# ShangHua-Gao/SOD100K

Measured on NVIDIA H100. Metric: images/sec CSNet fwd 224x224, higher is better.
Workload: dtype fp16

## Files before the change

### sod100k_b200/csrc/il_stream.cuh

```cuda
#pragma once
#include <cuda.h>

#include "il_block.cuh"

namespace csnet {

constexpr int kIlsMaxThreads = 768;
constexpr int kIlsMaxC = 64;
constexpr int kIlsHiStages = 2, kIlsLoStages = 3;

struct IlsArgs {
  void* yh;
  void* yl;
  const uint32_t* wh;
  const uint32_t* wl;
  DwParams dw1h, dw1l, dw2h, dw2l;
  float bias_h[kIlsMaxC], sm1_h[kIlsMaxC], bias_l[kIlsMaxC], sm1_l[kIlsMaxC];
  int32_t N, H, W;
  int32_t Chi, Cli, Cho, Clo;
  int32_t K8, K16, NH, NL;
  int32_t SH, SL, ST;
  int32_t GH, GL;
  int32_t ns, gsn, hl;
  int32_t GR, GLR;
  int32_t Ci, BW;
  int32_t off_xlo;
  int32_t cpi, total_chunks;
  int32_t dw_warps;
  int32_t hi_stage_bytes, lo_stage_bytes;
  int32_t off_xl, off_xh, off_t1l, off_wbh, off_wbl, off_bar, off_zero, off_epi, smem_bytes;
};

__device__ __forceinline__ void tma_load_5d(uint32_t dst, const CUtensorMap* tm, uint32_t bar, int c0, int c1, int c2, int c3, int c4) {
  asm volatile("cp.async.bulk.tensor.5d.shared::cluster.global.mbarrier::complete_tx::bytes [%0], [%1, {%3, %4, %5, %6, %7}], [%2];\n"
               ::"r"(dst), "l"(tm), "r"(bar), "r"(c0), "r"(c1), "r"(c2), "r"(c3), "r"(c4) : "memory");
}
__device__ __forceinline__ void tma_load_4d_a(uint32_t dst, const CUtensorMap* tm, uint32_t bar, int c0, int c1, int c2, int c3) {
  asm volatile("cp.async.bulk.tensor.4d.shared::cluster.global.mbarrier::complete_tx::bytes [%0], [%1, {%3, %4, %5, %6}], [%2];\n"
               ::"r"(dst), "l"(tm), "r"(bar), "r"(c0), "r"(c1), "r"(c2), "r"(c3) : "memory");
}
__device__ __forceinline__ void mbar_expect_tx_a(uint32_t bar, uint32_t bytes) {
  asm volatile("mbarrier.arrive.expect_tx.shared::cta.b64 _, [%0], %1;\n" ::"r"(bar), "r"(bytes) : "memory");
}
__device__ __forceinline__ void mbar_wait_a(uint32_t bar, uint32_t parity) {
  uint32_t ok = 0;
  const long long t0 = clock64();
  while (true) {
    asm volatile("{\n.reg .pred p;\nmbarrier.try_wait.parity.shared::cta.b64 p, [%1], %2;\nselp.u32 %0, 1, 0, p;\n}\n"
                 : "=r"(ok) : "r"(bar), "r"(parity) : "memory");
    if (ok) break;
    if (clock64() - t0 > 4000000000LL) __trap();
  }
}
__device__ __forceinline__ uint64_t gmma_desc(uint32_t saddr, uint32_t lbo_bytes, uint32_t sbo_bytes) {
  return (uint64_t)((saddr & 0x3FFFF) >> 4) | ((uint64_t)((lbo_bytes >> 4) & 0x3FFF) << 16) |
         ((uint64_t)((sbo_bytes >> 4) & 0x3FFF) << 32);
}
template <int N> struct Wgmma;
template <> struct Wgmma<16> {
  static __device__ __forceinline__ void mma(float (&d)[8], uint64_t da, uint64_t db, uint32_t acc) {
    asm volatile("{\n.reg .pred p;\nsetp.ne.b32 p, %10, 0;\n"
                 "wgmma.mma_async.sync.aligned.m64n16k16.f32.f16.f16 {%0, %1, %2, %3, %4, %5, %6, %7}, %8, %9, p, 1, 1, 1, 0;\n}\n"
                 : "+f"(d[0]), "+f"(d[1]), "+f"(d[2]), "+f"(d[3]), "+f"(d[4]), "+f"(d[5]), "+f"(d[6]), "+f"(d[7])
                 : "l"(da), "l"(db), "r"(acc));
  }
};
template <> struct Wgmma<32> {
  static __device__ __forceinline__ void mma(float (&d)[16], uint64_t da, uint64_t db, uint32_t acc) {
    asm volatile("{\n.reg .pred p;\nsetp.ne.b32 p, %18, 0;\n"
                 "wgmma.mma_async.sync.aligned.m64n32k16.f32.f16.f16 {%0, %1, %2, %3, %4, %5, %6, %7, %8, %9, %10, %11, %12, %13, %14, %15}, %16, %17, p, 1, 1, 1, 0;\n}\n"
                 : "+f"(d[0]), "+f"(d[1]), "+f"(d[2]), "+f"(d[3]), "+f"(d[4]), "+f"(d[5]), "+f"(d[6]), "+f"(d[7]), "+f"(d[8]), "+f"(d[9]), "+f"(d[10]), "+f"(d[11]), "+f"(d[12]), "+f"(d[13]), "+f"(d[14]), "+f"(d[15])
                 : "l"(da), "l"(db), "r"(acc));
  }
};
template <> struct Wgmma<48> {
  static __device__ __forceinline__ void mma(float (&d)[24], uint64_t da, uint64_t db, uint32_t acc) {
    asm volatile("{\n.reg .pred p;\nsetp.ne.b32 p, %26, 0;\n"
                 "wgmma.mma_async.sync.aligned.m64n48k16.f32.f16.f16 {%0, %1, %2, %3, %4, %5, %6, %7, %8, %9, %10, %11, %12, %13, %14, %15, %16, %17, %18, %19, %20, %21, %22, %23}, %24, %25, p, 1, 1, 1, 0;\n}\n"
                 : "+f"(d[0]), "+f"(d[1]), "+f"(d[2]), "+f"(d[3]), "+f"(d[4]), "+f"(d[5]), "+f"(d[6]), "+f"(d[7]), "+f"(d[8]), "+f"(d[9]), "+f"(d[10]), "+f"(d[11]), "+f"(d[12]), "+f"(d[13]), "+f"(d[14]), "+f"(d[15]), "+f"(d[16]), "+f"(d[17]), "+f"(d[18]), "+f"(d[19]), "+f"(d[20]), "+f"(d[21]), "+f"(d[22]), "+f"(d[23])
                 : "l"(da), "l"(db), "r"(acc));
  }
};
template <> struct Wgmma<64> {
  static __device__ __forceinline__ void mma(float (&d)[32], uint64_t da, uint64_t db, uint32_t acc) {
    asm volatile("{\n.reg .pred p;\nsetp.ne.b32 p, %34, 0;\n"
                 "wgmma.mma_async.sync.aligned.m64n64k16.f32.f16.f16 {%0, %1, %2, %3, %4, %5, %6, %7, %8, %9, %10, %11, %12, %13, %14, %15, %16, %17, %18, %19, %20, %21, %22, %23, %24, %25, %26, %27, %28, %29, %30, %31}, %32, %33, p, 1, 1, 1, 0;\n}\n"
                 : "+f"(d[0]), "+f"(d[1]), "+f"(d[2]), "+f"(d[3]), "+f"(d[4]), "+f"(d[5]), "+f"(d[6]), "+f"(d[7]), "+f"(d[8]), "+f"(d[9]), "+f"(d[10]), "+f"(d[11]), "+f"(d[12]), "+f"(d[13]), "+f"(d[14]), "+f"(d[15]), "+f"(d[16]), "+f"(d[17]), "+f"(d[18]), "+f"(d[19]), "+f"(d[20]), "+f"(d[21]), "+f"(d[22]), "+f"(d[23]), "+f"(d[24]), "+f"(d[25]), "+f"(d[26]), "+f"(d[27]), "+f"(d[28]), "+f"(d[29]), "+f"(d[30]), "+f"(d[31])
                 : "l"(da), "l"(db), "r"(acc));
  }
};
template <> struct Wgmma<80> {
  static __device__ __forceinline__ void mma(float (&d)[40], uint64_t da, uint64_t db, uint32_t acc) {
    asm volatile("{\n.reg .pred p;\nsetp.ne.b32 p, %42, 0;\n"
                 "wgmma.mma_async.sync.aligned.m64n80k16.f32.f16.f16 {%0, %1, %2, %3, %4, %5, %6, %7, %8, %9, %10, %11, %12, %13, %14, %15, %16, %17, %18, %19, %20, %21, %22, %23, %24, %25, %26, %27, %28, %29, %30, %31, %32, %33, %34, %35, %36, %37, %38, %39}, %40, %41, p, 1, 1, 1, 0;\n}\n"
                 : "+f"(d[0]), "+f"(d[1]), "+f"(d[2]), "+f"(d[3]), "+f"(d[4]), "+f"(d[5]), "+f"(d[6]), "+f"(d[7]), "+f"(d[8]), "+f"(d[9]), "+f"(d[10]), "+f"(d[11]), "+f"(d[12]), "+f"(d[13]), "+f"(d[14]), "+f"(d[15]), "+f"(d[16]), "+f"(d[17]), "+f"(d[18]), "+f"(d[19]), "+f"(d[20]), "+f"(d[21]), "+f"(d[22]), "+f"(d[23]), "+f"(d[24]), "+f"(d[25]), "+f"(d[26]), "+f"(d[27]), "+f"(d[28]), "+f"(d[29]), "+f"(d[30]), "+f"(d[31]), "+f"(d[32]), "+f"(d[33]), "+f"(d[34]), "+f"(d[35]), "+f"(d[36]), "+f"(d[37]), "+f"(d[38]), "+f"(d[39])
                 : "l"(da), "l"(db), "r"(acc));
  }
};
__device__ __forceinline__ void wgmma_fence() { asm volatile("wgmma.fence.sync.aligned;\n" ::: "memory"); }
__device__ __forceinline__ void wgmma_commit_wait() {
  asm volatile("wgmma.commit_group.sync.aligned;\n" ::: "memory");
  asm volatile("wgmma.wait_group.sync.aligned 0;\n" ::: "memory");
}
__device__ __forceinline__ void warpgroup_bar(int wg) { asm volatile("bar.sync %0, 128;\n" ::"r"(1 + wg) : "memory"); }
template <int N>
__device__ __forceinline__ void wgmma_block(float (&d)[N / 2], uint64_t da, uint64_t db, int K16) {
#pragma unroll
  for (int i = 0; i < N / 2; ++i) d[i] = 0.f;
  wgmma_fence();
  for (int ks = 0; ks < (K16 >> 4); ++ks) Wgmma<N>::mma(d, da + (uint64_t)(16 * ks), db + (uint64_t)(16 * ks), ks > 0);
  wgmma_commit_wait();
}
__device__ __forceinline__ uint32_t lds32(uint32_t a) { uint32_t v; asm volatile("ld.shared.b32 %0, [%1];\n" : "=r"(v) : "r"(a)); return v; }
__device__ __forceinline__ uint2 lds64(uint32_t a) { uint2 v; asm volatile("ld.shared.v2.b32 {%0, %1}, [%2];\n" : "=r"(v.x), "=r"(v.y) : "r"(a)); return v; }
__device__ __forceinline__ uint4 lds128(uint32_t a) {
  uint4 v;
  asm volatile("ld.shared.v4.b32 {%0, %1, %2, %3}, [%4];\n" : "=r"(v.x), "=r"(v.y), "=r"(v.z), "=r"(v.w) : "r"(a));
  return v;
}
__device__ __forceinline__ uint16_t lds16(uint32_t a) { uint16_t v; asm volatile("ld.shared.u16 %0, [%1];\n" : "=h"(v) : "r"(a)); return v; }
__device__ __forceinline__ void sts128(uint32_t a, uint4 v) {
  asm volatile("st.shared.v4.b32 [%0], {%1, %2, %3, %4};\n" ::"r"(a), "r"(v.x), "r"(v.y), "r"(v.z), "r"(v.w) : "memory");
}
__device__ __forceinline__ void sts16(uint32_t a, uint16_t v) { asm volatile("st.shared.u16 [%0], %1;\n" ::"r"(a), "h"(v) : "memory"); }

__device__ __forceinline__ uint16_t h16(const uint32_t* row, int j) { return (j & 1) ? (uint16_t)(row[j >> 1] >> 16) : (uint16_t)row[j >> 1]; }

template <typename T>
__device__ __forceinline__ void ils_dw_push(uint32_t (&t1)[2][6], uint32_t (&t2)[2][5], const uint32_t (&n1)[6],
                                            const uint32_t (&w1)[5], float b1, float s1, const uint32_t (&w2)[5], float b2, float s2,
                                            bool make_t2, float mL, float mR, bool make_out, uint16_t* out) {
  uint32_t q[5];
  if (make_t2) {
#pragma unroll
    for (int i = 0; i < 10; i += 2) {
      float v0 = b1, v1 = b1;
#pragma unroll
      for (int dy = 0; dy < 3; ++dy) {
        const uint32_t* row = dy == 0 ? t1[0] : (dy == 1 ? t1[1] : n1);
#pragma unroll
        for (int dx = 0; dx < 3; ++dx) {
          const uint16_t w = h16(w1, dy * 3 + dx);
          v0 = Pack<T>::fma16(h16(row, i + dx), w, v0);
          v1 = Pack<T>::fma16(h16(row, i + 1 + dx), w, v1);
        }
      }
      v0 = prelu_m1(v0, s1);
      v1 = prelu_m1(v1, s1);
      if (i == 0) v0 *= mL;
      if (i == 8) v1 *= mR;
      q[i >> 1] = Pack<T>::from_f2(v0, v1);
    }
  } else {
#pragma unroll
    for (int i = 0; i < 5; ++i) q[i] = 0u;
  }
  if (make_out) {
    uint32_t o[4];
#pragma unroll
    for (int k = 0; k < 8; k += 2) {
      float v0 = b2, v1 = b2;
#pragma unroll
      for (int dy = 0; dy < 3; ++dy) {
        const uint32_t* row = dy == 0 ? t2[0] : (dy == 1 ? t2[1] : q);
#pragma unroll
        for (int dx = 0; dx < 3; ++dx) {
          const uint16_t w = h16(w2, dy * 3 + dx);
          v0 = Pack<T>::fma16(h16(row, k + dx), w, v0);
          v1 = Pack<T>::fma16(h16(row, k + 1 + dx), w, v1);
        }
      }
      o[k >> 1] = Pack<T>::from_f2(prelu_m1(v0, s2), prelu_m1(v1, s2));
    }
    *reinterpret_cast<uint4*>(out) = make_uint4(o[0], o[1], o[2], o[3]);
  }
#pragma unroll
  for (int i = 0; i < 6; ++i) { t1[0][i] = t1[1][i]; t1[1][i] = n1[i]; }
#pragma unroll
  for (int i = 0; i < 5; ++i) { t2[0][i] = t2[1][i]; t2[1][i] = q[i]; }
}

__device__ __forceinline__ void stsm_x4_trans(uint32_t addr, uint32_t a, uint32_t b, uint32_t c, uint32_t d) {
  asm volatile("stmatrix.sync.aligned.m8n8.x4.trans.shared.b16 [%0], {%1, %2, %3, %4};\n" ::"r"(addr), "r"(a), "r"(b), "r"(c), "r"(d) : "memory");
}

template <typename T, int N>
__device__ __forceinline__ void ils_block(uint64_t da, uint64_t db, int K16, int wg, uint32_t tile, uint32_t gstride, int g0, int ngroups,
                                          uint32_t eb, uint32_t es, uint32_t dummy, int lane) {
  float d[N / 2];
  wgmma_block<N>(d, da, db, K16);
  warpgroup_bar(wg);
  const int q = lane & 3, mrow = lane & 7, mat = lane >> 3;
#pragma unroll
  for (int cc = 0; cc < N / 16; ++cc) {
    const uint32_t co = (uint32_t)(cc * 16 + 2 * q) * 4u;
    const uint2 bA = lds64(eb + co), bB = lds64(eb + co + 32u), sA = lds64(es + co), sB = lds64(es + co + 32u);
    const float b0 = __uint_as_float(bA.x), b1 = __uint_as_float(bA.y), b2 = __uint_as_float(bB.x), b3 = __uint_as_float(bB.y);
    const float s0 = __uint_as_float(sA.x), s1 = __uint_as_float(sA.y), s2 = __uint_as_float(sB.x), s3 = __uint_as_float(sB.y);
    const float* r = d + 8 * cc;
    const uint32_t m0 = Pack<T>::from_f2(prelu_m1(r[0] + b0, s0), prelu_m1(r[1] + b1, s1));
    const uint32_t m1 = Pack<T>::from_f2(prelu_m1(r[2] + b0, s0), prelu_m1(r[3] + b1, s1));
    const uint32_t m2 = Pack<T>::from_f2(prelu_m1(r[4] + b2, s2), prelu_m1(r[5] + b3, s3));
    const uint32_t m3 = Pack<T>::from_f2(prelu_m1(r[6] + b2, s2), prelu_m1(r[7] + b3, s3));
    const int pg = g0 + (mat & 1);
    const uint32_t addr = pg < ngroups ? tile + (uint32_t)pg * gstride + (uint32_t)(cc * 16 + 8 * (mat >> 1) + mrow) * 16u
                                       : dummy + (uint32_t)(mat * 8 + mrow) * 16u;
    stsm_x4_trans(addr, m0, m1, m2, m3);
  }
}
template <typename T>
__device__ __forceinline__ void ils_block_n(int N, uint64_t da, uint64_t db, int K16, int wg, uint32_t tile, uint32_t gstride, int g0,
                                            int ngroups, uint32_t eb, uint32_t es, uint32_t dummy, int lane) {
// ... 26 lines not shown
  if (tid == 0) {
    for (int i = 0; i < 6; ++i) asm volatile("mbarrier.init.shared::cta.b64 [%0], 1;\n" ::"r"(BAR + 8 * i) : "memory");
    asm volatile("fence.mbarrier_init.release.cluster;\n" ::: "memory");
  }
  {
    uint16_t* wb = reinterpret_cast<uint16_t*>(gbase + A.off_wbh);
    const uint16_t* src = reinterpret_cast<const uint16_t*>(A.wh);
    for (int i = tid; i < NH * K16; i += nthreads) {
      const int n = i / K16, k = i - n * K16;
      wb[(((n >> 3) * (K16 >> 3) + (k >> 3)) * 8 + (n & 7)) * 8 + (k & 7)] = k < A.K8 ? src[n * A.K8 + k] : (uint16_t)0;
    }
    if (NL > 0) {
      wb = reinterpret_cast<uint16_t*>(gbase + A.off_wbl);
      src = reinterpret_cast<const uint16_t*>(A.wl);
      for (int i = tid; i < NL * K16; i += nthreads) {
        const int n = i / K16, k = i - n * K16;
        wb[(((n >> 3) * (K16 >> 3) + (k >> 3)) * 8 + (n & 7)) * 8 + (k & 7)] = k < A.K8 ? src[n * A.K8 + k] : (uint16_t)0;
      }
    }
    if (tid < 16) reinterpret_cast<uint32_t*>(gbase + A.off_zero)[tid] = 0u;
    if (kStem) {
      const int per = K16 - Chi, padh = per * 4 * GR, padl = per * 2 * GLR;
      for (int i = tid; i < 2 * padh + padl; i += nthreads) {
        const bool hb = i < 2 * padh;
        const int st = hb ? i / padh : 0, j = hb ? i - st * padh : i - 2 * padh, g_ = j / per, k_ = Chi + (j - g_ * per);
        sts128((hb ? XH + (uint32_t)st * (uint32_t)A.hi_stage_bytes + (uint32_t)(g_ * SH + k_) * 16u
                   : sbase + A.off_xlo + (uint32_t)(g_ * SL + k_) * 16u), make_uint4(0u, 0u, 0u, 0u));
      }
    }
    if (tid < kIlsMaxC) {
      float* ep = reinterpret_cast<float*>(gbase + A.off_epi);
      ep[tid] = A.bias_h[tid]; ep[kIlsMaxC + tid] = A.sm1_h[tid]; ep[2 * kIlsMaxC + tid] = A.bias_l[tid]; ep[3 * kIlsMaxC + tid] = A.sm1_l[tid];
    }
  }
  asm volatile("fence.proxy.async.shared::cta;\n" ::: "memory");
  __syncthreads();

  const int n_hi_tasks = Cho * gsn;
  const bool dw_hi = tid < n_hi_tasks;
  const int dwt = dw_hi ? tid : tid - n_hi_tasks;
  const int Gd = dw_hi ? gsn : gsn >> 1, Cd = dw_hi ? Cho : Clo, Sd = dw_hi ? SH : ST;
  const bool dw_live = dwt < Cd * Gd;
  const int dc = dw_live ? dwt / Gd : 0, dg = dw_live ? dwt - dc * Gd : 0;
  uint32_t w1[5], w2[5];
  float b1, s1, b2, s2;
  {
    const DwParams& P1 = dw_hi ? A.dw1h : A.dw1l;
    const DwParams& P2 = dw_hi ? A.dw2h : A.dw2l;
    float f1[10], f2[10];
#pragma unroll
    for (int i = 0; i < 9; ++i) {
      f1[i] = dw_live ? __ldg(P1.w + dc * 9 + i) : 0.f;
      f2[i] = dw_live ? __ldg(P2.w + dc * 9 + i) : 0.f;
    }
    f1[9] = f2[9] = 0.f;
#pragma unroll
    for (int i = 0; i < 5; ++i) { w1[i] = Pack<T>::from_f2(f1[2 * i], f1[2 * i + 1]); w2[i] = Pack<T>::from_f2(f2[2 * i], f2[2 * i + 1]); }
    b1 = dw_live ? __ldg(P1.b + dc) : 0.f; s1 = dw_live ? __ldg(P1.s + dc) - 1.f : 0.f;
    b2 = dw_live ? __ldg(P2.b + dc) : 0.f; s2 = dw_live ? __ldg(P2.s + dc) - 1.f : 0.f;
  }
  const int dw_rows = dw_hi ? 4 : 2;
  const int dHd = dw_hi ? H : Hl, dWd = dw_hi ? W : Wl;
  const uint32_t dw_off = (uint32_t)((dg + hl) * Sd + dc) * 16u, dw_rowstep = (uint32_t)((dw_hi ? GR : GLR) * Sd) * 16u;
  const int Gimg = dw_hi ? GH : GL;

  const int nbh = (4 * GR + 7) >> 3, nbl = NL > 0 ? (2 * GLR + 7) >> 3 : 0;
  const uint64_t db_h = gmma_desc(WBH, 128u, (uint32_t)(K16 >> 3) * 128u), db_l = gmma_desc(WBL, 128u, (uint32_t)(K16 >> 3) * 128u);
  const uint32_t hi_tx = (uint32_t)(64 * SH * GR), lo_tx = kStem ? (uint32_t)(A.BW * 4 * A.Ci * 4) : (uint32_t)(32 * SL * GLR);
  const uint32_t XLO = sbase + A.off_xlo;

  int ra = (int)((long long)blockIdx.x * A.total_chunks / gridDim.x);
  const int rb = (int)((long long)(blockIdx.x + 1) * A.total_chunks / gridDim.x);
  uint32_t hq = 0, lq = 0;

  while (ra < rb) {
    const int item = ra / cpi, ca = ra - item * cpi;
    const int n = item / A.ns, gs0 = (item - n * A.ns) * gsn;
    const int cb = (ca + (rb - ra)) < cpi ? (ca + (rb - ra)) : cpi;
    ra += cb - ca;
    const int c0 = ca > 0 ? ca - 1 : 0, c1 = cb < cpi ? cb : cpi - 1;
    const int cl0 = c0 > 0 ? c0 - 1 : 0, cl1 = c1 + 1 < cpi ? c1 + 1 : cpi - 1;
    const int out_lo = dw_hi ? 4 * ca : 2 * ca, out_hi = dw_hi ? 4 * cb : 2 * cb;
    const uint32_t hq0 = hq, lq0 = lq;
    hq += (uint32_t)(c1 - c0 + 1);
    lq += (uint32_t)(cl1 - cl0 + 1);
    auto hi_stage = [&](int c) { return XH + ((hq0 + (uint32_t)(c - c0)) & 1u) * (uint32_t)A.hi_stage_bytes; };
    auto lo_stage = [&](int cl) { return XL + ((lq0 + (uint32_t)(cl - cl0)) % 3u) * (uint32_t)A.lo_stage_bytes; };
    auto issue_hi = [&](int c) {
      const uint32_t q = hq0 + (uint32_t)(c - c0), bar = bar_h + 8 * (q & 1u);
      mbar_expect_tx_a(bar, hi_tx);
      tma_load_5d(hi_stage(c), &tmH, bar, 0, 0, gs0 - hl, 4 * c, n);
    };
    auto issue_lo = [&](int cl) {
      const uint32_t q = lq0 + (uint32_t)(cl - cl0), bar = bar_l + 8 * (q % 3u);
      mbar_expect_tx_a(bar, lo_tx);
      if (kStem) tma_load_4d_a(lo_stage(cl), &tmL, bar, 8 * (gs0 - hl) - 4, 4 * cl, 0, n);
      else tma_load_5d(lo_stage(cl), &tmL, bar, 0, 0, (gs0 >> 1) - hl, 2 * cl, n);
    };
    if (tid == 0) {
      asm volatile("fence.proxy.async.shared::cta;\n" ::: "memory");
      if (!kStem) {
        issue_hi(c0);
        if (c0 + 1 <= c1) issue_hi(c0 + 1);
      }
      for (int cl = cl0; cl <= cl1 && cl <= c0 + 1; ++cl) issue_lo(cl);
    }
    int lo_waited = 0;
    uint32_t t1w[2][6], t2w[2][5];
#pragma unroll
    for (int i = 0; i < 6; ++i) t1w[0][i] = t1w[1][i] = 0u;
#pragma unroll
    for (int i = 0; i < 5; ++i) t2w[0][i] = t2w[1][i] = 0u;
    const int gimg = (dw_hi ? gs0 : gs0 >> 1) + dg;
    const bool edgeL = gimg == 0, edgeR = gimg == Gimg - 1;
    const float mL = edgeL ? 0.f : 1.f, mR = edgeR ? 0.f : 1.f;
    uint16_t* ybase = reinterpret_cast<uint16_t*>(dw_hi ? A.yh : A.yl) + ((size_t)n * Cd + dc) * dHd * dWd + 8 * gimg;

    for (int c = c0; c <= c1; ++c) {
      {
        const uint32_t q = hq0 + (uint32_t)(c - c0);
        if (!kStem) mbar_wait_a(bar_h + 8 * (q & 1u), (q >> 1) & 1u);
        const int need = (c + 1 < cpi ? c + 1 : cpi - 1) - cl0 + 1;
        while (lo_waited < need) {
          const uint32_t ql = lq0 + (uint32_t)lo_waited;
          mbar_wait_a(bar_l + 8 * (ql % 3u), (ql / 3u) & 1u);
          ++lo_waited;
        }
      }
      const uint32_t xh = hi_stage(c), xl = kStem ? XLO : lo_stage(c);
      if (kStem) {
        const int Ci = A.Ci, BW = A.BW;
        const int n_hi = 4 * GR * Ci * 3, n_lo = Clo > 0 ? 2 * GLR * Ci * 3 : 0;
        for (int task = tid; task < n_hi + n_lo; task += nthreads) {
          const bool hb = task < n_hi;
          const int t = hb ? task : task - n_hi, Gt = hb ? GR : GLR;
          const int ck = t % (Ci * 3), rg = t / (Ci * 3);
          const int ci = ck / 3, ky = ck - ci * 3, r = rg / Gt, g = rg - r * Gt;
          float f[10];
          if (hb) {
            const int yy = 4 * c + r + ky - 1;
            if (yy >= 0 && yy < H) {
              const uint32_t a = lo_stage(yy >> 2) + (uint32_t)(((ci * 4 + (yy & 3)) * BW + 8 * g + 3) * 4);
              const uint4 m0 = lds128(a + 4u), m1 = lds128(a + 20u);
              f[0] = __uint_as_float(lds32(a)); f[9] = __uint_as_float(lds32(a + 36u));
              f[1] = __uint_as_float(m0.x); f[2] = __uint_as_float(m0.y); f[3] = __uint_as_float(m0.z); f[4] = __uint_as_float(m0.w);
              f[5] = __uint_as_float(m1.x); f[6] = __uint_as_float(m1.y); f[7] = __uint_as_float(m1.z); f[8] = __uint_as_float(m1.w);
            } else {
#pragma unroll
// ... 84 lines not shown
                return __byte_perm(Pack<T>::max2(u, __byte_perm(u, 0u, 0x1032)), Pack<T>::max2(v, __byte_perm(v, 0u, 0x1032)), 0x5410);
              };
              uint4 o;
              o.x = hmax(Pack<T>::max2(a0.x, c0_.x), Pack<T>::max2(a0.y, c0_.y));
              o.y = hmax(Pack<T>::max2(a0.z, c0_.z), Pack<T>::max2(a0.w, c0_.w));
              o.z = hmax(Pack<T>::max2(a1.x, c1_.x), Pack<T>::max2(a1.y, c1_.y));
              o.w = hmax(Pack<T>::max2(a1.z, c1_.z), Pack<T>::max2(a1.w, c1_.w));
              sts128(dst + (uint32_t)(lr * GLR * SL) * 16u, o);
            }
          }
        }
      }
      asm volatile("fence.proxy.async.shared::cta;\n" ::: "memory");
      __syncthreads();
      if (warp == nwarps - 1 && lane == 0) {
        asm volatile("fence.proxy.async.shared::cta;\n" ::: "memory");
        if (!kStem && c >= c0 + 1 && c + 1 <= c1) issue_hi(c + 1);
        if (c + 2 <= cl1) issue_lo(c + 2);
      }
      if (warp < (nwarps & ~3)) {
        const int wg = warp >> 2, qd = warp & 3, wgs = nwarps >> 2;
        for (int b = wg; b < nbh + nbl; b += wgs) {
          if (b < nbh)
            ils_block_n<T>(NH, gmma_desc(xh + (uint32_t)(b * 8 * SH) * 16u, 128u, (uint32_t)SH * 16u), db_h, K16, wg, xh, (uint32_t)SH * 16u,
                           b * 8 + qd * 2, 4 * GR, EPI, EPI + 256u, DUMMY, lane);
          else
            ils_block_n<T>(NL, gmma_desc(xl + (uint32_t)((b - nbh) * 8 * SL) * 16u, 128u, (uint32_t)SL * 16u), db_l, K16, wg, T1L,
                           (uint32_t)ST * 16u, (b - nbh) * 8 + qd * 2, 2 * GLR, EPI + 512u, EPI + 768u, DUMMY, lane);
        }
      }
      __syncthreads();
      if (dw_live) {
        const uint32_t t1b = (dw_hi ? xh : T1L) + dw_off;
        for (int rr = 0; rr < dw_rows; ++rr) {
          const int r = dw_rows * c + rr;
          const uint32_t p = t1b + (uint32_t)rr * dw_rowstep;
          uint32_t n1[6];
          const uint4 m = lds128(p);
          n1[0] = lds32(edgeL ? ZERO : p - (uint32_t)Sd * 16u + 12u);
          n1[1] = m.x; n1[2] = m.y; n1[3] = m.z; n1[4] = m.w;
          n1[5] = lds32(edgeR ? ZERO : p + (uint32_t)Sd * 16u);
          const int tr = r - 1, orow = r - 2;
          const bool make_t2 = tr >= 0 && tr >= out_lo - 1 && tr <= out_hi;
          const bool make_out = orow >= out_lo && orow < out_hi;
          ils_dw_push<T>(t1w, t2w, n1, w1, b1, s1, w2, b2, s2, make_t2, mL, mR, make_out, ybase + (size_t)orow * dWd);
        }
      }
    }
    if (cb == cpi && dw_live) {
      const uint32_t z[6] = {0u, 0u, 0u, 0u, 0u, 0u};
      for (int rr = 0; rr < 2; ++rr) {
        const int r = dHd + rr, tr = r - 1, orow = r - 2;
        ils_dw_push<T>(t1w, t2w, z, w1, b1, s1, w2, b2, s2, tr < dHd, mL, mR, orow >= out_lo, ybase + (size_t)orow * dWd);
      }
    }
    __syncthreads();
  }
}

}
```

### sod100k_b200/csrc/plan.cu

```cuda
#include <cuda.h>
#include <cuda_runtime.h>

#include <cstdio>
#include <cstdlib>
#include <cstring>
#include <cstdint>
#include <new>
#include <string>
#include <vector>

#include "../../include/csnet_b200.h"
#include "generic_ops.cuh"
#include "il_block.cuh"
#include "il_stream.cuh"
#include "mix_stream.cuh"
#include "ms_direct.cuh"
#include "mix_tc.cuh"
#include "dw_fast.cuh"
#include "image_io.cuh"

namespace {

thread_local std::string g_err;

// ... 428 lines not shown
  EncodeTiledFn fn = encode_tiled_fn();
  if (!fn) return false;
  const cuuint64_t dims[4] = {(cuuint64_t)W, (cuuint64_t)H, (cuuint64_t)C, (cuuint64_t)N};
  const cuuint64_t strides[3] = {(cuuint64_t)W * 4, (cuuint64_t)H * W * 4, (cuuint64_t)C * H * W * 4};
  const cuuint32_t box[4] = {(cuuint32_t)bw, (cuuint32_t)rows, (cuuint32_t)bc, 1};
  const cuuint32_t estr[4] = {1, 1, 1, 1};
  return fn(tm, CU_TENSOR_MAP_DATA_TYPE_FLOAT32, 4, const_cast<void*>(base), dims, strides, box, estr,
            CU_TENSOR_MAP_INTERLEAVE_NONE, CU_TENSOR_MAP_SWIZZLE_NONE, CU_TENSOR_MAP_L2_PROMOTION_L2_128B,
            CU_TENSOR_MAP_FLOAT_OOB_FILL_NONE) == CUDA_SUCCESS;
}

bool plan_ils(const csnet_plan& P, const csnet_op_desc& op, const csnet::IlArgs& il, csnet::IlsArgs* out) {
  if (!P.ils_enabled || encode_tiled_fn() == nullptr) return false;
  const csnet_tensor_desc &Xh = P.tensors[op.paths[0].src], &Xl = P.tensors[op.paths[1].src], &Yh = P.tensors[op.dst];
  if (Yh.dtype != CSNET_F16) return false;
  const bool stem = op.paths[0].ksize == 3;
  csnet::IlsArgs A{};
  A.H = Yh.H; A.W = Yh.W;
  A.Chi = stem ? Xh.C * 9 : Xh.C; A.Cli = stem ? 0 : Xl.C; A.Cho = Yh.C; A.Clo = op.dst2 >= 0 ? P.tensors[op.dst2].C : 0;
  A.Ci = stem ? Xh.C : 0;
  if (stem && (Xh.dtype != CSNET_F32 || A.Chi > 32 || A.W % 4)) return false;
  if (A.W % 16 || A.H % 4 || A.Cho > csnet::kIlsMaxC || A.Clo > csnet::kIlsMaxC || A.Chi + A.Cli > 64) return false;
  A.K8 = stem ? 32 : round_up(A.Chi + A.Cli, 8);
  A.K16 = round_up(A.Chi + A.Cli, 16);
  A.NH = round_up(A.Cho, 16);
  A.NL = A.Clo > 0 ? round_up(A.Clo, 16) : 0;
  A.GH = A.W / 8; A.GL = A.W / 16;
  A.SH = (A.K16 > A.NH ? A.K16 : A.NH) + 1;
  A.SL = A.Clo > 0 ? A.K16 + 1 : (A.Cli | 1);
  A.ST = A.NL + 1;
  A.cpi = A.H / 4;
  auto r128 = [](int v) { return (v + 127) / 128 * 128; };
  bool found = false;
  double best_cost = 0;
  csnet::IlsArgs best{};
  for (int ns = 1; ns <= 16; ++ns) {
    if (P.ils_force_ns > 0 && ns != P.ils_force_ns) continue;
    if (A.GH % ns || (A.GH / ns) % 2) continue;
    csnet::IlsArgs T = A;
    T.ns = ns; T.gsn = A.GH / ns; T.hl = ns > 1 ? 1 : 0;
    T.GR = T.gsn + 2 * T.hl; T.GLR = T.gsn / 2 + 2 * T.hl;
    T.dw_warps = (T.Cho * T.gsn + T.Clo * (T.gsn / 2) + 31) / 32;
    if (T.dw_warps < 4) T.dw_warps = 4;
    const int warps = T.dw_warps;
    if (warps * 32 > csnet::kIlsMaxThreads || T.SH > 256 || T.SL > 256 || T.GR > 256) continue;
    const int nbh = (4 * T.GR + 7) / 8, nbl = T.Clo > 0 ? (2 * T.GLR + 7) / 8 : 0;
    T.BW = 8 * T.GR + 8;
    if (stem && T.BW > 256) continue;
    T.lo_stage_bytes = stem ? r128(T.BW * 4 * T.Ci * 4) : r128(2 * T.GLR * T.SL * 16);
    T.hi_stage_bytes = r128(4 * T.GR * T.SH * 16);
    T.off_xl = 0;
    T.off_xh = csnet::kIlsLoStages * T.lo_stage_bytes;
    T.off_t1l = T.off_xh + csnet::kIlsHiStages * T.hi_stage_bytes;
    T.off_wbh = T.off_t1l + r128(2 * T.GLR * T.ST * 16);
    T.off_wbl = T.off_wbh + r128(T.NH * T.K16 * 2);
    T.off_bar = T.off_wbl + r128(T.NL * T.K16 * 2);
    T.off_zero = T.off_bar + 256;
    T.off_epi = T.off_zero + 128;
    T.off_xlo = T.off_epi + 1536;
    int end = T.off_xlo + (stem ? r128(2 * T.GLR * T.SL * 16) : 0);
    const int over_h = T.off_xh + T.hi_stage_bytes + nbh * 8 * T.SH * 16,
              over_l = (stem ? T.off_xlo : T.off_xl + 2 * T.lo_stage_bytes) + nbl * 8 * T.SL * 16;
    end = over_h > end ? over_h : end;
    end = over_l > end ? over_l : end;
    T.smem_bytes = end + 128;
    if (T.smem_bytes > 227 * 1024) continue;
    const double cost = 0.55 + 0.45 * T.GR / T.gsn;
    if (!found || cost < best_cost) { best = T; best_cost = cost; found = true; }
  }
  if (!found) return false;
  best.wh = il.wh; best.wl = il.wl;
  best.dw1h = il.dw1h; best.dw1l = il.dw1l; best.dw2h = il.dw2h; best.dw2l = il.dw2l;
  *out = best;
  return true;
}

bool is_msd(const csnet_plan& P, const csnet_op_desc& op) {
  if (op.kind != CSNET_OP_MIX || op.ext_off[23] == 1 || op.n_paths < 1) return false;
  const csnet_tensor_desc& D = P.tensors[op.dst];
  if (D.dtype != CSNET_F16 || D.W % 8) return false;
  for (int p = 0; p < op.n_paths; ++p) {
    const csnet_path_desc& q = op.paths[p];
    const csnet_tensor_desc& S = P.tensors[q.src];
    if (q.ksize != 3 || q.src != op.paths[0].src || q.c0 != 0 || q.cin != S.C || q.stride != 1 || q.pad != q.dil || q.pool != 1 || q.pre_avg ||
        q.up != 1 || S.dtype != CSNET_F16 || S.H != D.H || S.W != D.W || q.cout > 8 || q.cin > 128)
      return false;
    if (q.dil != 1 && q.dil != 2 && q.dil != 4 && q.dil != 8 && q.dil != 16) return false;
  }
  return true;
}

bool plan_ms(const csnet_plan& P, const csnet_op_desc& op, csnet::MsArgs* out) {
  if (!P.ms_enabled || encode_tiled_fn() == nullptr) return false;
  if (op.kind == CSNET_OP_MIX && op.ext_off[23] == 1) return false;
  const csnet_tensor_desc& D = P.tensors[op.dst];
  csnet::MsArgs A{};
  A.C = mix_channels(P, op);
  A.has_proj = op.kind == CSNET_OP_MIXPROJ;
  if (A.C > csnet::kMsMaxC || D.W % 8 || D.H % csnet::kMsRows) return false;
  if (A.has_proj ? D.dtype != CSNET_F32 : D.dtype == CSNET_BF16) return false;
  A.dst_f32 = D.dtype == CSNET_F32;
// ... 861 lines not shown
```

Baseline: 13960.

## Restructure IL depthwise stage to process two groups per thread with fp32 sliding accumulators

Each depthwise thread now handles two adjacent 8-pixel groups (16 outputs) and keeps running fp32 partial sums across rows, with per-channel weights staged in shared memory instead of packed fp16 registers. The dw thread count is halved, the max threads cap is lowered, and the plan now takes the first feasible split instead of the cost-minimizing one. The first wgmma of each block also skips accumulator zeroing. This cuts redundant halo loads and per-row recomputation, but raises register pressure and changes the tile selection, which may pick a worse split.

```diff
diff --git a/sod100k_b200/csrc/il_stream.cuh b/sod100k_b200/csrc/il_stream.cuh
--- a/sod100k_b200/csrc/il_stream.cuh
+++ b/sod100k_b200/csrc/il_stream.cuh
@@ -5,7 +5,7 @@
 
 namespace csnet {
 
-constexpr int kIlsMaxThreads = 768;
+constexpr int kIlsMaxThreads = 384;
 constexpr int kIlsMaxC = 64;
 constexpr int kIlsHiStages = 2, kIlsLoStages = 3;
 
@@ -28,7 +28,7 @@
   int32_t cpi, total_chunks;
   int32_t dw_warps;
   int32_t hi_stage_bytes, lo_stage_bytes;
-  int32_t off_xl, off_xh, off_t1l, off_wbh, off_wbl, off_bar, off_zero, off_epi, smem_bytes;
+  int32_t off_xl, off_xh, off_t1l, off_wbh, off_wbl, off_bar, off_zero, off_epi, off_dwp, smem_bytes;
 };
 
 __device__ __forceinline__ void tma_load_5d(uint32_t dst, const CUtensorMap* tm, uint32_t bar, int c0, int c1, int c2, int c3, int c4) {
@@ -64,6 +64,12 @@
                  : "+f"(d[0]), "+f"(d[1]), "+f"(d[2]), "+f"(d[3]), "+f"(d[4]), "+f"(d[5]), "+f"(d[6]), "+f"(d[7])
                  : "l"(da), "l"(db), "r"(acc));
   }
+  static __device__ __forceinline__ void mma0(float (&d)[8], uint64_t da, uint64_t db) {
+    asm volatile("{\n.reg .pred p;\nsetp.ne.b32 p, %10, 0;\n"
+                 "wgmma.mma_async.sync.aligned.m64n16k16.f32.f16.f16 {%0, %1, %2, %3, %4, %5, %6, %7}, %8, %9, p, 1, 1, 1, 0;\n}\n"
+                 : "=f"(d[0]), "=f"(d[1]), "=f"(d[2]), "=f"(d[3]), "=f"(d[4]), "=f"(d[5]), "=f"(d[6]), "=f"(d[7])
+                 : "l"(da), "l"(db), "r"(0u));
+  }
 };
 template <> struct Wgmma<32> {
   static __device__ __forceinline__ void mma(float (&d)[16], uint64_t da, uint64_t db, uint32_t acc) {
@@ -72,6 +78,12 @@
                  : "+f"(d[0]), "+f"(d[1]), "+f"(d[2]), "+f"(d[3]), "+f"(d[4]), "+f"(d[5]), "+f"(d[6]), "+f"(d[7]), "+f"(d[8]), "+f"(d[9]), "+f"(d[10]), "+f"(d[11]), "+f"(d[12]), "+f"(d[13]), "+f"(d[14]), "+f"(d[15])
                  : "l"(da), "l"(db), "r"(acc));
   }
+  static __device__ __forceinline__ void mma0(float (&d)[16], uint64_t da, uint64_t db) {
+    asm volatile("{\n.reg .pred p;\nsetp.ne.b32 p, %18, 0;\n"
+                 "wgmma.mma_async.sync.aligned.m64n32k16.f32.f16.f16 {%0, %1, %2, %3, %4, %5, %6, %7, %8, %9, %10, %11, %12, %13, %14, %15}, %16, %17, p, 1, 1, 1, 0;\n}\n"
+                 : "=f"(d[0]), "=f"(d[1]), "=f"(d[2]), "=f"(d[3]), "=f"(d[4]), "=f"(d[5]), "=f"(d[6]), "=f"(d[7]), "=f"(d[8]), "=f"(d[9]), "=f"(d[10]), "=f"(d[11]), "=f"(d[12]), "=f"(d[13]), "=f"(d[14]), "=f"(d[15])
+                 : "l"(da), "l"(db), "r"(0u));
+  }
 };
 template <> struct Wgmma<48> {
   static __device__ __forceinline__ void mma(float (&d)[24], uint64_t da, uint64_t db, uint32_t acc) {
@@ -80,6 +92,12 @@
                  : "+f"(d[0]), "+f"(d[1]), "+f"(d[2]), "+f"(d[3]), "+f"(d[4]), "+f"(d[5]), "+f"(d[6]), "+f"(d[7]), "+f"(d[8]), "+f"(d[9]), "+f"(d[10]), "+f"(d[11]), "+f"(d[12]), "+f"(d[13]), "+f"(d[14]), "+f"(d[15]), "+f"(d[16]), "+f"(d[17]), "+f"(d[18]), "+f"(d[19]), "+f"(d[20]), "+f"(d[21]), "+f"(d[22]), "+f"(d[23])
                  : "l"(da), "l"(db), "r"(acc));
   }
+  static __device__ __forceinline__ void mma0(float (&d)[24], uint64_t da, uint64_t db) {
+    asm volatile("{\n.reg .pred p;\nsetp.ne.b32 p, %26, 0;\n"
+                 "wgmma.mma_async.sync.aligned.m64n48k16.f32.f16.f16 {%0, %1, %2, %3, %4, %5, %6, %7, %8, %9, %10, %11, %12, %13, %14, %15, %16, %17, %18, %19, %20, %21, %22, %23}, %24, %25, p, 1, 1, 1, 0;\n}\n"
+                 : "=f"(d[0]), "=f"(d[1]), "=f"(d[2]), "=f"(d[3]), "=f"(d[4]), "=f"(d[5]), "=f"(d[6]), "=f"(d[7]), "=f"(d[8]), "=f"(d[9]), "=f"(d[10]), "=f"(d[11]), "=f"(d[12]), "=f"(d[13]), "=f"(d[14]), "=f"(d[15]), "=f"(d[16]), "=f"(d[17]), "=f"(d[18]), "=f"(d[19]), "=f"(d[20]), "=f"(d[21]), "=f"(d[22]), "=f"(d[23])
+                 : "l"(da), "l"(db), "r"(0u));
+  }
 };
 template <> struct Wgmma<64> {
   static __device__ __forceinline__ void mma(float (&d)[32], uint64_t da, uint64_t db, uint32_t acc) {
@@ -88,6 +106,12 @@
                  : "+f"(d[0]), "+f"(d[1]), "+f"(d[2]), "+f"(d[3]), "+f"(d[4]), "+f"(d[5]), "+f"(d[6]), "+f"(d[7]), "+f"(d[8]), "+f"(d[9]), "+f"(d[10]), "+f"(d[11]), "+f"(d[12]), "+f"(d[13]), "+f"(d[14]), "+f"(d[15]), "+f"(d[16]), "+f"(d[17]), "+f"(d[18]), "+f"(d[19]), "+f"(d[20]), "+f"(d[21]), "+f"(d[22]), "+f"(d[23]), "+f"(d[24]), "+f"(d[25]), "+f"(d[26]), "+f"(d[27]), "+f"(d[28]), "+f"(d[29]), "+f"(d[30]), "+f"(d[31])
                  : "l"(da), "l"(db), "r"(acc));
   }
+  static __device__ __forceinline__ void mma0(float (&d)[32], uint64_t da, uint64_t db) {
+    asm volatile("{\n.reg .pred p;\nsetp.ne.b32 p, %34, 0;\n"
+                 "wgmma.mma_async.sync.aligned.m64n64k16.f32.f16.f16 {%0, %1, %2, %3, %4, %5, %6, %7, %8, %9, %10, %11, %12, %13, %14, %15, %16, %17, %18, %19, %20, %21, %22, %23, %24, %25, %26, %27, %28, %29, %30, %31}, %32, %33, p, 1, 1, 1, 0;\n}\n"
+                 : "=f"(d[0]), "=f"(d[1]), "=f"(d[2]), "=f"(d[3]), "=f"(d[4]), "=f"(d[5]), "=f"(d[6]), "=f"(d[7]), "=f"(d[8]), "=f"(d[9]), "=f"(d[10]), "=f"(d[11]), "=f"(d[12]), "=f"(d[13]), "=f"(d[14]), "=f"(d[15]), "=f"(d[16]), "=f"(d[17]), "=f"(d[18]), "=f"(d[19]), "=f"(d[20]), "=f"(d[21]), "=f"(d[22]), "=f"(d[23]), "=f"(d[24]), "=f"(d[25]), "=f"(d[26]), "=f"(d[27]), "=f"(d[28]), "=f"(d[29]), "=f"(d[30]), "=f"(d[31])
+                 : "l"(da), "l"(db), "r"(0u));
+  }
 };
 template <> struct Wgmma<80> {
   static __device__ __forceinline__ void mma(float (&d)[40], uint64_t da, uint64_t db, uint32_t acc) {
@@ -96,6 +120,12 @@
                  : "+f"(d[0]), "+f"(d[1]), "+f"(d[2]), "+f"(d[3]), "+f"(d[4]), "+f"(d[5]), "+f"(d[6]), "+f"(d[7]), "+f"(d[8]), "+f"(d[9]), "+f"(d[10]), "+f"(d[11]), "+f"(d[12]), "+f"(d[13]), "+f"(d[14]), "+f"(d[15]), "+f"(d[16]), "+f"(d[17]), "+f"(d[18]), "+f"(d[19]), "+f"(d[20]), "+f"(d[21]), "+f"(d[22]), "+f"(d[23]), "+f"(d[24]), "+f"(d[25]), "+f"(d[26]), "+f"(d[27]), "+f"(d[28]), "+f"(d[29]), "+f"(d[30]), "+f"(d[31]), "+f"(d[32]), "+f"(d[33]), "+f"(d[34]), "+f"(d[35]), "+f"(d[36]), "+f"(d[37]), "+f"(d[38]), "+f"(d[39])
                  : "l"(da), "l"(db), "r"(acc));
   }
+  static __device__ __forceinline__ void mma0(float (&d)[40], uint64_t da, uint64_t db) {
+    asm volatile("{\n.reg .pred p;\nsetp.ne.b32 p, %42, 0;\n"
+                 "wgmma.mma_async.sync.aligned.m64n80k16.f32.f16.f16 {%0, %1, %2, %3, %4, %5, %6, %7, %8, %9, %10, %11, %12, %13, %14, %15, %16, %17, %18, %19, %20, %21, %22, %23, %24, %25, %26, %27, %28, %29, %30, %31, %32, %33, %34, %35, %36, %37, %38, %39}, %40, %41, p, 1, 1, 1, 0;\n}\n"
+                 : "=f"(d[0]), "=f"(d[1]), "=f"(d[2]), "=f"(d[3]), "=f"(d[4]), "=f"(d[5]), "=f"(d[6]), "=f"(d[7]), "=f"(d[8]), "=f"(d[9]), "=f"(d[10]), "=f"(d[11]), "=f"(d[12]), "=f"(d[13]), "=f"(d[14]), "=f"(d[15]), "=f"(d[16]), "=f"(d[17]), "=f"(d[18]), "=f"(d[19]), "=f"(d[20]), "=f"(d[21]), "=f"(d[22]), "=f"(d[23]), "=f"(d[24]), "=f"(d[25]), "=f"(d[26]), "=f"(d[27]), "=f"(d[28]), "=f"(d[29]), "=f"(d[30]), "=f"(d[31]), "=f"(d[32]), "=f"(d[33]), "=f"(d[34]), "=f"(d[35]), "=f"(d[36]), "=f"(d[37]), "=f"(d[38]), "=f"(d[39])
+                 : "l"(da), "l"(db), "r"(0u));
+  }
 };
 __device__ __forceinline__ void wgmma_fence() { asm volatile("wgmma.fence.sync.aligned;\n" ::: "memory"); }
 __device__ __forceinline__ void wgmma_commit_wait() {
@@ -105,10 +135,9 @@
 __device__ __forceinline__ void warpgroup_bar(int wg) { asm volatile("bar.sync %0, 128;\n" ::"r"(1 + wg) : "memory"); }
 template <int N>
 __device__ __forceinline__ void wgmma_block(float (&d)[N / 2], uint64_t da, uint64_t db, int K16) {
-#pragma unroll
-  for (int i = 0; i < N / 2; ++i) d[i] = 0.f;
   wgmma_fence();
-  for (int ks = 0; ks < (K16 >> 4); ++ks) Wgmma<N>::mma(d, da + (uint64_t)(16 * ks), db + (uint64_t)(16 * ks), ks > 0);
+  Wgmma<N>::mma0(d, da, db);
+  for (int ks = 1; ks < (K16 >> 4); ++ks) Wgmma<N>::mma(d, da + (uint64_t)(16 * ks), db + (uint64_t)(16 * ks), 1u);
   wgmma_commit_wait();
 }
 __device__ __forceinline__ uint32_t lds32(uint32_t a) { uint32_t v; asm volatile("ld.shared.b32 %0, [%1];\n" : "=r"(v) : "r"(a)); return v; }
@@ -126,58 +155,81 @@
 
 __device__ __forceinline__ uint16_t h16(const uint32_t* row, int j) { return (j & 1) ? (uint16_t)(row[j >> 1] >> 16) : (uint16_t)row[j >> 1]; }
 
+constexpr int kIlsDwpBytes = 96;
+constexpr int kIlsTX = 20, kIlsT2 = 18, kIlsTO = 16;
+
+template <int NO, bool kStart = false>
+__device__ __forceinline__ void ils_dw_taps(float (&acc)[NO], const float* row, float4 w) {
+#pragma unroll
+  for (int i = 0; i < NO; ++i) {
+    acc[i] = fmaf(row[i], w.x, kStart ? w.w : acc[i]);
+    acc[i] = fmaf(row[i + 1], w.y, acc[i]);
+    acc[i] = fmaf(row[i + 2], w.z, acc[i]);
+  }
+}
+__device__ __forceinline__ float4 ils_dw_param(uint32_t a) {
+  const uint4 v = lds128(a);
+  return make_float4(__uint_as_float(v.x), __uint_as_float(v.y), __uint_as_float(v.z), __uint_as_float(v.w));
+}
+struct IlsTail {
+  float s2a[kIlsT2], s2b[kIlsT2];
+  float soa[kIlsTO], sob[kIlsTO];
+};
+__device__ __forceinline__ void ils_dw_start(IlsTail& t, uint32_t prm) {
+  float z0;
+  asm("mov.b32 %0, 0;\n" : "=f"(z0));
+  float z[kIlsTX];
+#pragma unroll
+  for (int i = 0; i < kIlsTX; ++i) z[i] = z0;
+  float4 w0 = ils_dw_param(prm), w1 = ils_dw_param(prm + 16u);
+  ils_dw_taps<kIlsT2, true>(t.s2a, z, w0); ils_dw_taps<kIlsT2>(t.s2a, z, w1); ils_dw_taps<kIlsT2, true>(t.s2b, z, w0);
+  w0 = ils_dw_param(prm + 48u); w1 = ils_dw_param(prm + 64u);
+  ils_dw_taps<kIlsTO, true>(t.soa, z, w0); ils_dw_taps<kIlsTO>(t.soa, z, w1); ils_dw_taps<kIlsTO, true>(t.sob, z, w0);
+}
+struct IlsTaskEdges {
+  float m0, m9, m17;
+  bool outB;
+};
 template <typename T>
-__device__ __forceinline__ void ils_dw_push(uint32_t (&t1)[2][6], uint32_t (&t2)[2][5], const uint32_t (&n1)[6],
-                                            const uint32_t (&w1)[5], float b1, float s1, const uint32_t (&w2)[5], float b2, float s2,
-                                            bool make_t2, float mL, float mR, bool make_out, uint16_t* out) {
-  uint32_t q[5];
-  if (make_t2) {
-#pragma unroll
-    for (int i = 0; i < 10; i += 2) {
-      float v0 = b1, v1 = b1;
-#pragma unroll
-      for (int dy = 0; dy < 3; ++dy) {
-        const uint32_t* row = dy == 0 ? t1[0] : (dy == 1 ? t1[1] : n1);
-#pragma unroll
-        for (int dx = 0; dx < 3; ++dx) {
-          const uint16_t w = h16(w1, dy * 3 + dx);
-          v0 = Pack<T>::fma16(h16(row, i + dx), w, v0);
-          v1 = Pack<T>::fma16(h16(row, i + 1 + dx), w, v1);
-        }
-      }
-      v0 = prelu_m1(v0, s1);
-      v1 = prelu_m1(v1, s1);
-      if (i == 0) v0 *= mL;
-      if (i == 8) v1 *= mR;
-      q[i >> 1] = Pack<T>::from_f2(v0, v1);
-    }
-  } else {
-#pragma unroll
-    for (int i = 0; i < 5; ++i) q[i] = 0u;
-  }
+__device__ __forceinline__ void ils_dw_push(float (&s2a)[kIlsT2], float (&s2b)[kIlsT2], float (&soa)[kIlsTO], float (&sob)[kIlsTO],
+                                            const float (&x)[kIlsTX], uint32_t prm, bool make_t2, const IlsTaskEdges& e, bool make_out,
+                                            uint16_t* out) {
+  ils_dw_taps<kIlsT2>(s2a, x, ils_dw_param(prm + 32u));
+  const float4 w1 = ils_dw_param(prm + 16u);
+  float q[kIlsT2];
+#pragma unroll
+  for (int i = 0; i < kIlsT2; i += 2) {
+    float v0 = prelu_m1(s2a[i], w1.w), v1 = prelu_m1(s2a[i + 1], w1.w);
+    if (i == 0) v0 *= e.m0;
+    if (i == 8) v1 *= e.m9;
+    if (i == 16) v1 *= e.m17;
+    const float2 r = Pack<T>::to_f2(Pack<T>::from_f2(v0, v1));
+    q[i] = make_t2 ? r.x : 0.f;
+    q[i + 1] = make_t2 ? r.y : 0.f;
+  }
+  ils_dw_taps<kIlsT2>(s2b, x, w1);
+  ils_dw_taps<kIlsTO>(soa, q, ils_dw_param(prm + 80u));
+  const float4 v1 = ils_dw_param(prm + 64u);
+  ils_dw_taps<kIlsTO>(sob, q, v1);
   if (make_out) {
-    uint32_t o[4];
-#pragma unroll
-    for (int k = 0; k < 8; k += 2) {
-      float v0 = b2, v1 = b2;
-#pragma unroll
-      for (int dy = 0; dy < 3; ++dy) {
-        const uint32_t* row = dy == 0 ? t2[0] : (dy == 1 ? t2[1] : q);
-#pragma unroll
-        for (int dx = 0; dx < 3; ++dx) {
-          const uint16_t w = h16(w2, dy * 3 + dx);
-          v0 = Pack<T>::fma16(h16(row, k + dx), w, v0);
-          v1 = Pack<T>::fma16(h16(row, k + 1 + dx), w, v1);
-        }
-      }
-      o[k >> 1] = Pack<T>::from_f2(prelu_m1(v0, s2), prelu_m1(v1, s2));
-    }
+    uint32_t o[8];
+#pragma unroll
+    for (int k = 0; k < kIlsTO; k += 2) o[k >> 1] = Pack<T>::from_f2(prelu_m1(soa[k], v1.w), prelu_m1(soa[k + 1], v1.w));
     *reinterpret_cast<uint4*>(out) = make_uint4(o[0], o[1], o[2], o[3]);
-  }
-#pragma unroll
-  for (int i = 0; i < 6; ++i) { t1[0][i] = t1[1][i]; t1[1][i] = n1[i]; }
-#pragma unroll
-  for (int i = 0; i < 5; ++i) { t2[0][i] = t2[1][i]; t2[1][i] = q[i]; }
+    if (e.outB) *reinterpret_cast<uint4*>(out + 8) = make_uint4(o[4], o[5], o[6], o[7]);
+  }
+  ils_dw_taps<kIlsTO, true>(soa, q, ils_dw_param(prm + 48u));
+  ils_dw_taps<kIlsT2, true>(s2a, x, ils_dw_param(prm));
+}
+template <typename T>
+__device__ __forceinline__ void ils_dw_load(float (&x)[kIlsTX], uint32_t pA, uint32_t pB, uint32_t pL, uint32_t pR) {
+  const uint4 a = lds128(pA), b = lds128(pB);
+  const uint32_t u[10] = {lds32(pL), a.x, a.y, a.z, a.w, b.x, b.y, b.z, b.w, lds32(pR)};
+#pragma unroll
+  for (int i = 0; i < 10; ++i) {
+    const float2 f = Pack<T>::to_f2(u[i]);
+    x[2 * i] = f.x; x[2 * i + 1] = f.y;
+  }
 }
 
 __device__ __forceinline__ void stsm_x4_trans(uint32_t addr, uint32_t a, uint32_t b, uint32_t c, uint32_t d) {
@@ -270,33 +322,30 @@
       float* ep = reinterpret_cast<float*>(gbase + A.off_epi);
       ep[tid] = A.bias_h[tid]; ep[kIlsMaxC + tid] = A.sm1_h[tid]; ep[2 * kIlsMaxC + tid] = A.bias_l[tid]; ep[3 * kIlsMaxC + tid] = A.sm1_l[tid];
     }
+    float* dp = reinterpret_cast<float*>(gbase + A.off_dwp);
+    for (int i = tid; i < (Cho + Clo) * 24; i += nthreads) {
+      const int ch = i / 24, j = i - ch * 24, lyr = j / 12, dy = (j >> 2) % 3, k = j & 3;
+      const bool hi = ch < Cho;
+      const int cc = hi ? ch : ch - Cho;
+      const DwParams& P = lyr ? (hi ? A.dw2h : A.dw2l) : (hi ? A.dw1h : A.dw1l);
+      float v = 0.f;
+      if (k < 3) v = Pack<T>::to_f2(Pack<T>::from_f2(__ldg(P.w + cc * 9 + dy * 3 + k), 0.f)).x;
+      else if (dy == 0) v = __ldg(P.b + cc);
+      else if (dy == 1) v = __ldg(P.s + cc) - 1.f;
+      dp[i] = v;
+    }
   }
   asm volatile("fence.proxy.async.shared::cta;\n" ::: "memory");
   __syncthreads();
 
-  const int n_hi_tasks = Cho * gsn;
+  const int n_hi_tasks = Cho * (gsn >> 1);
   const bool dw_hi = tid < n_hi_tasks;
   const int dwt = dw_hi ? tid : tid - n_hi_tasks;
-  const int Gd = dw_hi ? gsn : gsn >> 1, Cd = dw_hi ? Cho : Clo, Sd = dw_hi ? SH : ST;
+  const int Gs = dw_hi ? gsn : gsn >> 1;
+  const int Gd = (Gs + 1) >> 1, Cd = dw_hi ? Cho : Clo, Sd = dw_hi ? SH : ST;
   const bool dw_live = dwt < Cd * Gd;
-  const int dc = dw_live ? dwt / Gd : 0, dg = dw_live ? dwt - dc * Gd : 0;
-  uint32_t w1[5], w2[5];
-  float b1, s1, b2, s2;
-  {
-    const DwParams& P1 = dw_hi ? A.dw1h : A.dw1l;
-    const DwParams& P2 = dw_hi ? A.dw2h : A.dw2l;
-    float f1[10], f2[10];
-#pragma unroll
-    for (int i = 0; i < 9; ++i) {
-      f1[i] = dw_live ? __ldg(P1.w + dc * 9 + i) : 0.f;
-      f2[i] = dw_live ? __ldg(P2.w + dc * 9 + i) : 0.f;
-    }
-    f1[9] = f2[9] = 0.f;
-#pragma unroll
-    for (int i = 0; i < 5; ++i) { w1[i] = Pack<T>::from_f2(f1[2 * i], f1[2 * i + 1]); w2[i] = Pack<T>::from_f2(f2[2 * i], f2[2 * i + 1]); }
-    b1 = dw_live ? __ldg(P1.b + dc) : 0.f; s1 = dw_live ? __ldg(P1.s + dc) - 1.f : 0.f;
-    b2 = dw_live ? __ldg(P2.b + dc) : 0.f; s2 = dw_live ? __ldg(P2.s + dc) - 1.f : 0.f;
-  }
+  const int dc = dw_live ? dwt / Gd : 0, dg = dw_live ? 2 * (dwt - dc * Gd) : 0;
+  const uint32_t prm = sbase + A.off_dwp + (uint32_t)((dw_hi ? dc : Cho + dc) * kIlsDwpBytes);
   const int dw_rows = dw_hi ? 4 : 2;
   const int dHd = dw_hi ? H : Hl, dWd = dw_hi ? W : Wl;
   const uint32_t dw_off = (uint32_t)((dg + hl) * Sd + dc) * 16u, dw_rowstep = (uint32_t)((dw_hi ? GR : GLR) * Sd) * 16u;
@@ -344,14 +393,16 @@
       for (int cl = cl0; cl <= cl1 && cl <= c0 + 1; ++cl) issue_lo(cl);
     }
     int lo_waited = 0;
-    uint32_t t1w[2][6], t2w[2][5];
-#pragma unroll
-    for (int i = 0; i < 6; ++i) t1w[0][i] = t1w[1][i] = 0u;
-#pragma unroll
-    for (int i = 0; i < 5; ++i) t2w[0][i] = t2w[1][i] = 0u;
+    IlsTail tl;
+    if (dw_live) ils_dw_start(tl, prm);
     const int gimg = (dw_hi ? gs0 : gs0 >> 1) + dg;
-    const bool edgeL = gimg == 0, edgeR = gimg == Gimg - 1;
-    const float mL = edgeL ? 0.f : 1.f, mR = edgeR ? 0.f : 1.f;
+    const bool hasB = gimg + 1 < Gimg, zeroL = gimg == 0, zeroR = gimg + 2 >= Gimg || dg + 2 >= Gs + hl;
+    IlsTaskEdges edg;
+    edg.m0 = zeroL ? 0.f : 1.f;
+    edg.m9 = hasB ? 1.f : 0.f;
+    edg.m17 = gimg + 2 >= Gimg ? 0.f : 1.f;
+    edg.outB = dg + 1 < Gs;
+    const uint32_t sd = (uint32_t)Sd * 16u;
     uint16_t* ybase = reinterpret_cast<uint16_t*>(dw_hi ? A.yh : A.yl) + ((size_t)n * Cd + dc) * dHd * dWd + 8 * gimg;
 
     for (int c = c0; c <= c1; ++c) {
@@ -502,27 +553,27 @@
       __syncthreads();
       if (dw_live) {
         const uint32_t t1b = (dw_hi ? xh : T1L) + dw_off;
-        for (int rr = 0; rr < dw_rows; ++rr) {
-          const int r = dw_rows * c + rr;
-          const uint32_t p = t1b + (uint32_t)rr * dw_rowstep;
-          uint32_t n1[6];
-          const uint4 m = lds128(p);
-          n1[0] = lds32(edgeL ? ZERO : p - (uint32_t)Sd * 16u + 12u);
-          n1[1] = m.x; n1[2] = m.y; n1[3] = m.z; n1[4] = m.w;
-          n1[5] = lds32(edgeR ? ZERO : p + (uint32_t)Sd * 16u);
-          const int tr = r - 1, orow = r - 2;
+        auto row = [&](float (&a2)[kIlsT2], float (&b2)[kIlsT2], float (&ao)[kIlsTO], float (&bo)[kIlsTO], int rr) {
+          const int r = dw_rows * c + rr, tr = r - 1, orow = r - 2;
           const bool make_t2 = tr >= 0 && tr >= out_lo - 1 && tr <= out_hi;
           const bool make_out = orow >= out_lo && orow < out_hi;
-          ils_dw_push<T>(t1w, t2w, n1, w1, b1, s1, w2, b2, s2, make_t2, mL, mR, make_out, ybase + (size_t)orow * dWd);
+          const uint32_t p = t1b + (uint32_t)rr * dw_rowstep;
+          float x[kIlsTX];
+          ils_dw_load<T>(x, p, hasB ? p + sd : ZERO, zeroL ? ZERO : p - sd + 12u, zeroR ? ZERO : p + 2u * sd);
+          ils_dw_push<T>(a2, b2, ao, bo, x, prm, make_t2, edg, make_out, ybase + (size_t)orow * dWd);
+        };
+        for (int rr = 0; rr < dw_rows; rr += 2) {
+          row(tl.s2a, tl.s2b, tl.soa, tl.sob, rr);
+          row(tl.s2b, tl.s2a, tl.sob, tl.soa, rr + 1);
         }
       }
     }
     if (cb == cpi && dw_live) {
-      const uint32_t z[6] = {0u, 0u, 0u, 0u, 0u, 0u};
-      for (int rr = 0; rr < 2; ++rr) {
-        const int r = dHd + rr, tr = r - 1, orow = r - 2;
-        ils_dw_push<T>(t1w, t2w, z, w1, b1, s1, w2, b2, s2, tr < dHd, mL, mR, orow >= out_lo, ybase + (size_t)orow * dWd);
-      }
+      float z[kIlsTX];
+#pragma unroll
+      for (int i = 0; i < kIlsTX; ++i) z[i] = 0.f;
+      ils_dw_push<T>(tl.s2a, tl.s2b, tl.soa, tl.sob, z, prm, true, edg, dHd - 2 >= out_lo, ybase + (size_t)(dHd - 2) * dWd);
+      ils_dw_push<T>(tl.s2b, tl.s2a, tl.sob, tl.soa, z, prm, false, edg, dHd - 1 >= out_lo, ybase + (size_t)(dHd - 1) * dWd);
     }
     __syncthreads();
   }
diff --git a/sod100k_b200/csrc/plan.cu b/sod100k_b200/csrc/plan.cu
--- a/sod100k_b200/csrc/plan.cu
+++ b/sod100k_b200/csrc/plan.cu
@@ -484,7 +484,6 @@
   A.cpi = A.H / 4;
   auto r128 = [](int v) { return (v + 127) / 128 * 128; };
   bool found = false;
-  double best_cost = 0;
   csnet::IlsArgs best{};
   for (int ns = 1; ns <= 16; ++ns) {
     if (P.ils_force_ns > 0 && ns != P.ils_force_ns) continue;
@@ -492,7 +491,7 @@
     csnet::IlsArgs T = A;
     T.ns = ns; T.gsn = A.GH / ns; T.hl = ns > 1 ? 1 : 0;
     T.GR = T.gsn + 2 * T.hl; T.GLR = T.gsn / 2 + 2 * T.hl;
-    T.dw_warps = (T.Cho * T.gsn + T.Clo * (T.gsn / 2) + 31) / 32;
+    T.dw_warps = (T.Cho * (T.gsn / 2) + T.Clo * ((T.gsn / 2 + 1) / 2) + 31) / 32;
     if (T.dw_warps < 4) T.dw_warps = 4;
     const int warps = T.dw_warps;
     if (warps * 32 > csnet::kIlsMaxThreads || T.SH > 256 || T.SL > 256 || T.GR > 256) continue;
@@ -509,7 +508,8 @@
     T.off_bar = T.off_wbl + r128(T.NL * T.K16 * 2);
     T.off_zero = T.off_bar + 256;
     T.off_epi = T.off_zero + 128;
-    T.off_xlo = T.off_epi + 1536;
+    T.off_dwp = T.off_epi + 1536;
+    T.off_xlo = T.off_dwp + r128((T.Cho + T.Clo) * csnet::kIlsDwpBytes);
     int end = T.off_xlo + (stem ? r128(2 * T.GLR * T.SL * 16) : 0);
     const int over_h = T.off_xh + T.hi_stage_bytes + nbh * 8 * T.SH * 16,
               over_l = (stem ? T.off_xlo : T.off_xl + 2 * T.lo_stage_bytes) + nbl * 8 * T.SL * 16;
@@ -517,8 +517,9 @@
     end = over_l > end ? over_l : end;
     T.smem_bytes = end + 128;
     if (T.smem_bytes > 227 * 1024) continue;
-    const double cost = 0.55 + 0.45 * T.GR / T.gsn;
-    if (!found || cost < best_cost) { best = T; best_cost = cost; found = true; }
+    best = T;
+    found = true;
+    break;
   }
   if (!found) return false;
   best.wh = il.wh; best.wl = il.wl;
```

New measurement: 16520 (median of 6 runs). +18.4%, better.
